# octavian-ganea/equidock_public

Measured on NVIDIA H100. Metric: protein_pairs_per_sec_iegmn_fwd_kabsch, higher is better.
Workload: dtype f32

## Files before the change

equidock_public_b200/csrc/attn_tc.cu:

```cuda
#include "tc_common.cuh"

namespace eqd {

#define AT_THREADS 256
#define AT_KEYS 64
#define AT_CHUNK_BYTES 8192
#define AT_A_SPLIT 16384
#define AT_LD 68

struct AtGroupSmem {
  unsigned char k[2][3][AT_CHUNK_BYTES];
  unsigned char v[2][3][AT_CHUNK_BYTES];
  float red[EQD_TM * 2];
  float x5c[2][AT_KEYS * 16];
  float red5[EQD_TM * 2 * 5];
};
struct AtSmem {
  unsigned char qa[3 * AT_A_SPLIT];
  unsigned char pa[3 * AT_A_SPLIT];
  AtGroupSmem grp;
  unsigned long long k_bar[2], v_bar[2];
};

__global__ void __launch_bounds__(AT_THREADS, 1)
attention0_tc_kernel(eqd_graph g, const float* __restrict__ proj, int pw, const unsigned char* __restrict__ kv,
                    long kv_split_stride, const float* __restrict__ x5, float* __restrict__ mu, int ldmu) {
  extern __shared__ __align__(128) unsigned char smem_raw[];
  AtSmem& S = *reinterpret_cast<AtSmem*>(smem_raw);
  const int tid = threadIdx.x, q = tid, half = q >> 7, r = q & 127, wgi = tid >> 7;
  AtGroupSmem& G = S.grp;
  if (tid == 0) {
    for (int b = 0; b < 2; ++b) {
      mbar_init(&S.k_bar[b], 1);
      mbar_init(&S.v_bar[b], 1);
    }
    asm volatile("fence.mbarrier_init.release.cluster;" ::: "memory");
  }
  __syncthreads();
  const unsigned k_saddr = smem_u32(G.k), v_saddr = smem_u32(G.v);
  const unsigned qa_saddr = smem_u32(S.qa), pa_saddr = smem_u32(S.pa);
  float* const dtile = reinterpret_cast<float*>(S.pa);
  unsigned kph[2] = {0, 0}, vph[2] = {0, 0};
  const int B = g.n_pairs;
  const unsigned char* k_g = kv;
  const unsigned char* v_g = kv + 3 * kv_split_stride;

  auto load_chunk = [&](const unsigned char* src, unsigned char (*dst)[AT_CHUNK_BYTES], unsigned long long* bar, int blk0,
                        int x5buf) {
    if (q == 0) {
      const bool with5 = x5buf >= 0;
      mbar_expect_tx(bar, 3 * AT_CHUNK_BYTES + (with5 ? AT_KEYS * 64 : 0));
#pragma unroll
      for (int s = 0; s < 3; ++s) bulk_g2s(dst[s], src + s * kv_split_stride + (long)blk0 * 1024, AT_CHUNK_BYTES, bar);
      if (with5) bulk_g2s(G.x5c[x5buf], x5 + (long)blk0 * 8 * 16, AT_KEYS * 64, bar);
    }
  };
  auto add_s5 = [&](float (&s)[32], const float* xc, const float (&q5)[5]) {
#pragma unroll
    for (int i = 0; i < 32; ++i) {
      const float* row = xc + (half * 32 + i) * 16;
      const float4 k4 = *reinterpret_cast<const float4*>(row);
      const float k8 = row[8];
      s[i] += q5[0] * k4.x + q5[1] * k4.y + q5[2] * k4.z + q5[3] * k4.w + q5[4] * k8;
    }
  };
  auto gemm_s = [&](int kb_, bool hi_only) {
    float d[32];
    wg_gemm6<64>(d, [&](int sp, int kb) { return a_desc_at<EQD_TM>(qa_saddr, AT_A_SPLIT, wgi, sp, kb); },
                 [&](int sp, int kk) { return b_desc_ex(k_saddr + (kb_ * 3 + sp) * AT_CHUNK_BYTES + kk * 256, 128, 1024); },
                 4, false, hi_only);
    wg_store_d<64>(dtile + wgi * 64 * AT_LD, AT_LD, d, tid & 127);
  };
  auto gemm_pv = [&](int vb_) {
    float d[32];
    wg_gemm6<64, 1>(d, [&](int sp, int kb) { return a_desc_at<EQD_TM>(pa_saddr, AT_A_SPLIT, wgi, sp, kb); },
                    [&](int sp, int kk) { return b_desc_ex(v_saddr + (vb_ * 3 + sp) * AT_CHUNK_BYTES + kk * 2048, 1024, 128); },
                    4, false);
    __syncthreads();
    wg_store_d<64>(dtile + wgi * 64 * AT_LD, AT_LD, d, tid & 127);
  };

  for (int tile = blockIdx.x; tile < g.n_node_tiles; tile += gridDim.x) {
    const int seg = g.node_tiles[2 * tile], node0 = g.node_tiles[2 * tile + 1];
    const int nvalid = min(EQD_TM, g.seg_ptr[seg + 1] - node0);
    const int pseg = seg < B ? seg + B : seg - B;
    const int j0 = g.seg_ptr[pseg], j1 = g.seg_ptr[pseg + 1];
    const int blk_lo = j0 >> 3, blk_hi = (j1 + 7) >> 3;
    const int nchunks = (blk_hi - blk_lo + 7) >> 3;
    const int node = node0 + r;
    const bool valid = r < nvalid;
    if (nchunks > 0) load_chunk(k_g, G.k[0], &S.k_bar[0], blk_lo, 0);
    float q5[5] = {0.f, 0.f, 0.f, 0.f, 0.f};
    if (valid) {
#pragma unroll
      for (int e = 0; e < 5; ++e) q5[e] = x5[(long)node * 16 + 10 + e];
    }
    {
      float v[32];
      const float4* sp = reinterpret_cast<const float4*>(proj + (long)node * pw + 128 + half * 32);
#pragma unroll
      for (int c4 = 0; c4 < 8; ++c4) {
        float4 t = valid ? sp[c4] : make_float4(0.f, 0.f, 0.f, 0.f);
        v[c4 * 4] = t.x; v[c4 * 4 + 1] = t.y; v[c4 * 4 + 2] = t.z; v[c4 * 4 + 3] = t.w;
      }
      store_half_split3<EQD_TM>(S.qa, AT_A_SPLIT, r, half * 32, v);
    }
    tc_fence_before();
    __syncthreads();
    float mx = -INFINITY;
    for (int c = 0; c < nchunks; ++c) {
      const int kb_ = c & 1;
      mbar_wait(&S.k_bar[kb_], kph[kb_]);
      kph[kb_] ^= 1;
      if (c + 1 < nchunks) load_chunk(k_g, G.k[kb_ ^ 1], &S.k_bar[kb_ ^ 1], blk_lo + 8 * (c + 1), kb_ ^ 1);
      else load_chunk(k_g, G.k[kb_ ^ 1], &S.k_bar[kb_ ^ 1], blk_lo, kb_ ^ 1);
      gemm_s(kb_, true);
      __syncthreads();
      float s[32];
      tile_ld32f(dtile, AT_LD, r, half * 32, s);
      add_s5(s, G.x5c[kb_], q5);
      const int key0 = (blk_lo + 8 * c) * 8 + half * 32;
#pragma unroll
      for (int i = 0; i < 32; ++i) {
        int kn = key0 + i;
        mx = fmaxf(mx, (kn >= j0 && kn < j1) ? s[i] : -INFINITY);
      }
      __syncthreads();
    }
    G.red[r * 2 + half] = mx;
    __syncthreads();
    mx = fmaxf(G.red[r * 2], G.red[r * 2 + 1]);
    float l = 0.f;
    float o_acc[32];
#pragma unroll
    for (int i = 0; i < 32; ++i) o_acc[i] = 0.f;
    if (nchunks > 0) load_chunk(v_g, G.v[0], &S.v_bar[0], blk_lo, -1);
    float o5[5] = {0.f, 0.f, 0.f, 0.f, 0.f};
    for (int c = 0; c < nchunks; ++c) {
      const int kb_ = (nchunks + c) & 1, vb_ = c & 1;
      mbar_wait(&S.k_bar[kb_], kph[kb_]);
      kph[kb_] ^= 1;
      if (c + 1 < nchunks) {
        load_chunk(k_g, G.k[kb_ ^ 1], &S.k_bar[kb_ ^ 1], blk_lo + 8 * (c + 1), kb_ ^ 1);
        load_chunk(v_g, G.v[vb_ ^ 1], &S.v_bar[vb_ ^ 1], blk_lo + 8 * (c + 1), -1);
      }
      gemm_s(kb_, false);
      __syncthreads();
      float s[32];
      tile_ld32f(dtile, AT_LD, r, half * 32, s);
      add_s5(s, G.x5c[kb_], q5);
      const int key0 = (blk_lo + 8 * c) * 8 + half * 32;
      float l4[4] = {0.f, 0.f, 0.f, 0.f};
#pragma unroll
      for (int i = 0; i < 32; ++i) {
        int kn = key0 + i;
        float pj = (kn >= j0 && kn < j1) ? expf(s[i] - mx) : 0.f;
        s[i] = pj;
        l4[i & 3] += pj;
        {
          const float* row = G.x5c[kb_] + (half * 32 + i) * 16;
          const float4 v4 = *reinterpret_cast<const float4*>(row + 4);
          o5[0] = fmaf(pj, v4.x, o5[0]);
          o5[1] = fmaf(pj, v4.y, o5[1]);
          o5[2] = fmaf(pj, v4.z, o5[2]);
          o5[3] = fmaf(pj, v4.w, o5[3]);
          o5[4] = fmaf(pj, row[9], o5[4]);
        }
      }
      l += (l4[0] + l4[1]) + (l4[2] + l4[3]);
      __syncthreads();
      store_half_split3<EQD_TM>(S.pa, AT_A_SPLIT, r, half * 32, s);
      tc_fence_before();
      __syncthreads();
      mbar_wait(&S.v_bar[vb_], vph[vb_]);
      vph[vb_] ^= 1;
      gemm_pv(vb_);
      __syncthreads();
      {
        float oc[32];
        tile_ld32f(dtile, AT_LD, r, half * 32, oc);
#pragma unroll
        for (int i = 0; i < 32; ++i) o_acc[i] += oc[i];
      }
      __syncthreads();
    }
    G.red[r * 2 + half] = l;
    {
#pragma unroll
      for (int e = 0; e < 5; ++e) G.red5[(r * 2 + half) * 5 + e] = o5[e];
    }
    __syncthreads();
    l = G.red[r * 2] + G.red[r * 2 + 1];
    {
      const float inv = l > 0.f ? 1.f / l : 0.f;
      if (valid && half == 0) {
        float e8[8];
#pragma unroll
        for (int e = 0; e < 5; ++e) e8[e] = (G.red5[r * 10 + e] + G.red5[r * 10 + 5 + e]) * inv;
        e8[5] = e8[6] = e8[7] = 0.f;
        float4* de = reinterpret_cast<float4*>(mu + (long)node * ldmu + 64);
        de[0] = make_float4(e8[0], e8[1], e8[2], e8[3]);
        de[1] = make_float4(e8[4], e8[5], e8[6], e8[7]);
      }
      if (valid) {
        float4* dst = reinterpret_cast<float4*>(mu + (long)node * ldmu + half * 32);
#pragma unroll
        for (int c4 = 0; c4 < 8; ++c4)
          dst[c4] = make_float4(o_acc[c4 * 4] * inv, o_acc[c4 * 4 + 1] * inv, o_acc[c4 * 4 + 2] * inv, o_acc[c4 * 4 + 3] * inv);
      }
    }
    __syncthreads();
  }
}

#define AT_CHAINS 2

struct __align__(128) AtChainSmem {
  unsigned char k[2][3][AT_CHUNK_BYTES];
  unsigned char v[2][3][AT_CHUNK_BYTES];
  float qs[64 * 64];
  unsigned long long k_bar[2], v_bar[2];
};

struct AtTile {
  int node0, nvalid;
  int j0, j1;
  int blk_lo, nchunks;
};

template <int P>
__global__ void __launch_bounds__(AT_CHAINS * 128, 1)
attention64_tc_kernel(eqd_graph g, const float* __restrict__ proj, const unsigned char* __restrict__ kv,
                      long kv_split_stride, float* __restrict__ mu) {
  extern __shared__ __align__(128) unsigned char smem_raw[];
  AtChainSmem& W = reinterpret_cast<AtChainSmem*>(smem_raw)[threadIdx.x >> 7];
  const int tid = threadIdx.x, wgi = tid >> 7, t = tid & 127, lane = t & 31;
  const int bar = 1 + wgi;
  if (t == 0) {
    for (int b = 0; b < 2; ++b) {
      mbar_init(&W.k_bar[b], 1);
      mbar_init(&W.v_bar[b], 1);
    }
    asm volatile("fence.mbarrier_init.release.cluster;" ::: "memory");
  }
  wg_barrier(bar);
  const unsigned k_saddr = smem_u32(W.k), v_saddr = smem_u32(W.v);
  const int B = g.n_pairs, nht = 2 * g.n_node_tiles, hstride = gridDim.x * AT_CHAINS;
  const unsigned char* k_g = kv;
  const unsigned char* v_g = kv + 3 * kv_split_stride;

  const int chain = blockIdx.x * AT_CHAINS + wgi;
  auto find_tile = [&](int k, AtTile& m) {
    for (; chain + k * hstride < nht; ++k) {
      const int ht = (chain + k * hstride) ^ (k & 1);
      const int seg = __ldg(g.node_tiles + 2 * (ht >> 1));
      m.node0 = __ldg(g.node_tiles + 2 * (ht >> 1) + 1) + 64 * (ht & 1);
      m.nvalid = min(64, __ldg(g.seg_ptr + seg + 1) - m.node0);
      if (m.nvalid <= 0) continue;
      const int pseg = seg < B ? seg + B : seg - B;
      m.j0 = __ldg(g.seg_ptr + pseg);
      m.j1 = __ldg(g.seg_ptr + pseg + 1);
      m.blk_lo = m.j0 >> 3;
      m.nchunks = (((m.j1 + 7) >> 3) - m.blk_lo + 7) >> 3;
      return k;
    }
    return -1;
  };
  unsigned kfill = 0, kcons = 0, vfill = 0, vcons = 0;
  auto fill = [&](unsigned char (*dst)[3][AT_CHUNK_BYTES], unsigned long long* bars, unsigned& n, const unsigned char* src,
                  int blk0) {
    if (t == 0) {
      unsigned long long* b = &bars[n & 1];
      mbar_expect_tx(b, 3 * AT_CHUNK_BYTES);
#pragma unroll
      for (int s = 0; s < 3; ++s) bulk_g2s(dst[n & 1][s], src + s * kv_split_stride + (long)blk0 * 1024, AT_CHUNK_BYTES, b);
    }
    ++n;
  };
  auto consume = [&](unsigned long long* bars, unsigned& n) {
    mbar_wait(&bars[n & 1], (n >> 1) & 1);
    return (int)((n++) & 1);
  };
  auto stage_q = [&](const AtTile& m) { stage_rows64(W.qs, proj, 320, 128, m.node0, m.nvalid, t); };

  const int fr0 = (t >> 5) * 16 + (lane >> 2), fc = 2 * (lane & 3);
  AtTile cur, nxt;
  int kt = find_tile(0, cur);
  bool k_ahead = false, v_ahead = false;
  if (kt >= 0) stage_q(cur);
  while (kt >= 0) {
    int ktn = -1;
    bool looked = false;
    auto look_ahead = [&]() {
      if (looked) return;
      looked = true;
      ktn = find_tile(kt + 1, nxt);
      if (ktn >= 0) stage_q(nxt);
    };
    if (cur.nchunks > 0 && !k_ahead) fill(W.k, W.k_bar, kfill, k_g, cur.blk_lo);
    cp_async_wait<0>();
    wg_barrier(bar);
    unsigned qf[3][4][4];
    staged_rows_to_a_split3<P>(W.qs, t, qf);
    wg_barrier(bar);
    auto k_desc = [&](int kb_) {
      return [&, kb_](int sp, int kk) { return b_desc_ex(k_saddr + (kb_ * 3 + sp) * AT_CHUNK_BYTES + kk * 256, 128, 1024); };
    };
    float mx[2] = {-INFINITY, -INFINITY};
    for (int c = 0; c < cur.nchunks; ++c) {
      const int kb_ = consume(W.k_bar, kcons);
      fill(W.k, W.k_bar, kfill, k_g, cur.blk_lo + (c + 1 < cur.nchunks ? 8 * (c + 1) : 0));
      float s[32];
      wg_gemm6_rs_issue<64, 4, 0, true>(s, qf, k_desc(kb_), false);
      look_ahead();
      wg_mma_wait(s);
      const int key0 = (cur.blk_lo + 8 * c) * 8 + fc;
#pragma unroll
      for (int j = 0; j < 8; ++j)
#pragma unroll
        for (int e = 0; e < 2; ++e) {
          const int kn = key0 + 8 * j + e;
          const bool ok = kn >= cur.j0 && kn < cur.j1;
#pragma unroll
          for (int h = 0; h < 2; ++h) mx[h] = fmaxf(mx[h], ok ? s[4 * j + 2 * h + e] : -INFINITY);
        }
      wg_barrier(bar);
    }
    look_ahead();
#pragma unroll
    for (int h = 0; h < 2; ++h) {
      mx[h] = fmaxf(mx[h], __shfl_xor_sync(0xffffffffu, mx[h], 1));
      mx[h] = fmaxf(mx[h], __shfl_xor_sync(0xffffffffu, mx[h], 2));
    }
    float lh[2][2] = {{0.f, 0.f}, {0.f, 0.f}};
    float o_acc[32];
#pragma unroll
    for (int i = 0; i < 32; ++i) o_acc[i] = 0.f;
    if (cur.nchunks > 0 && !v_ahead) fill(W.v, W.v_bar, vfill, v_g, cur.blk_lo);
    for (int c = 0; c < cur.nchunks; ++c) {
      const int kb_ = consume(W.k_bar, kcons);
      const bool last = c + 1 == cur.nchunks;
      if (!last) {
        fill(W.k, W.k_bar, kfill, k_g, cur.blk_lo + 8 * (c + 1));
        fill(W.v, W.v_bar, vfill, v_g, cur.blk_lo + 8 * (c + 1));
      } else if (ktn >= 0 && nxt.nchunks > 0) {
        fill(W.k, W.k_bar, kfill, k_g, nxt.blk_lo);
        fill(W.v, W.v_bar, vfill, v_g, nxt.blk_lo);
      }
      float s[32];
      wg_gemm6_rs_issue<64, 4, 0, false, P>(s, qf, k_desc(kb_), false);
      wg_mma_wait(s);
      const int key0 = (cur.blk_lo + 8 * c) * 8 + fc;
#pragma unroll
      for (int j = 0; j < 8; ++j)
#pragma unroll
        for (int e = 0; e < 2; ++e) {
          const int kn = key0 + 8 * j + e;
          const bool ok = kn >= cur.j0 && kn < cur.j1;
#pragma unroll
          for (int h = 0; h < 2; ++h) {
            float& x = s[4 * j + 2 * h + e];
            x = ok ? expf(x - mx[h]) : 0.f;
          }
        }
      {
        float ps[32];
#pragma unroll
        for (int i = 0; i < 32; ++i) ps[i] = __shfl_xor_sync(0xffffffffu, s[i], 2);
#pragma unroll
        for (int h = 0; h < 2; ++h)
#pragma unroll
          for (int ch = 0; ch < 2; ++ch) {
            float s0 = 0.f, s1 = 0.f;
#pragma unroll
            for (int c4 = 0; c4 < 8; ++c4) {
              s0 = __fadd_rn(s0, chain_val(s, ps, h, ch, c4, 0));
              s1 = __fadd_rn(s1, chain_val(s, ps, h, ch, c4, 1));
            }
            const float sp = __fadd_rn(s0, s1);
            lh[h][ch] = __fadd_rn(lh[h][ch], __fadd_rn(sp, __shfl_xor_sync(0xffffffffu, sp, 1)));
          }
      }
      unsigned pf[3][4][4];
      acc_to_a_split3<4, P>(s, pf);
      const int vb_ = consume(W.v_bar, vcons);
      float o[32];
      wg_gemm6_rs_issue<64, 4, 1, false, P>(o, pf, [&](int sp, int kk) {
        return b_desc_ex(v_saddr + (vb_ * 3 + sp) * AT_CHUNK_BYTES + kk * 2048, 1024, 128); }, false);
      wg_mma_wait(o);
#pragma unroll
      for (int i = 0; i < 32; ++i) o_acc[i] = __fadd_rn(o_acc[i], o[i]);
      wg_barrier(bar);
    }
    k_ahead = v_ahead = ktn >= 0 && nxt.nchunks > 0 && cur.nchunks > 0;
#pragma unroll
    for (int h = 0; h < 2; ++h) {
      const float l = __fadd_rn(lh[h][0], lh[h][1]);
      const float inv = l > 0.f ? 1.f / l : 0.f;
      const int row = fr0 + 8 * h;
      if (row < cur.nvalid) {
        float* dst = mu + (long)(cur.node0 + row) * EQD_HID + fc;
#pragma unroll
        for (int j = 0; j < 8; ++j)
          *reinterpret_cast<float2*>(dst + 8 * j) = make_float2(o_acc[4 * j + 2 * h] * inv, o_acc[4 * j + 2 * h + 1] * inv);
      }
    }
    kt = ktn;
    cur = nxt;
  }
  cp_async_wait<0>();
}

template <int P>
static int launch_attention64_tc(const eqd_graph* g, const float* proj, const void* kv, float* mu, void* stream) {
  const size_t smem = AT_CHAINS * sizeof(AtChainSmem);
  EQD_SET_SMEM(attention64_tc_kernel<P>, smem);
  const int nht = 2 * g->n_node_tiles;
  int grid = (nht + AT_CHAINS - 1) / AT_CHAINS;
  if (grid > EQD_SMS) grid = EQD_SMS;
  const long split_stride = (long)((g->n_nodes + 7) / 8 + 8) * 1024;
  attention64_tc_kernel<P><<<grid, AT_CHAINS * 128, smem, (cudaStream_t)stream>>>(
      *g, proj, reinterpret_cast<const unsigned char*>(kv), split_stride, mu);
  EQD_CUDA_LAUNCH_CHECK();
  return EQD_OK;
}

}

int eqd_attention_tc_products(const eqd_graph* g, const float* proj, const void* kv, float* mu, int products, void* stream) {
  if (!g || !proj || !kv || !mu) return EQD_ERR_BAD_ARG;
  if (reinterpret_cast<uintptr_t>(kv) & 15) return EQD_ERR_BAD_ARG;
  if (products != 6 && products != 3) return EQD_ERR_UNSUPPORTED;
  if (g->n_node_tiles <= 0) return EQD_OK;
  return products == 3 ? eqd::launch_attention64_tc<3>(g, proj, kv, mu, stream)
                       : eqd::launch_attention64_tc<6>(g, proj, kv, mu, stream);
}

extern "C" int eqd_attention_tc(const eqd_graph* g, const float* proj, const void* kv, float* mu, void* stream) {
  return eqd_attention_tc_products(g, proj, kv, mu, 6, stream);
}

extern "C" int eqd_attention_tc0(const eqd_graph* g, const float* proj, const void* kv, const float* x5, float* mu,
                                 void* stream) {
  if (!g || !proj || !kv || !x5 || !mu) return EQD_ERR_BAD_ARG;
  if ((reinterpret_cast<uintptr_t>(kv) | reinterpret_cast<uintptr_t>(x5)) & 15) return EQD_ERR_BAD_ARG;
  if (g->n_node_tiles <= 0) return EQD_OK;
  const size_t smem = sizeof(eqd::AtSmem) + 128;
  EQD_SET_SMEM(eqd::attention0_tc_kernel, smem);
  const int grid = g->n_node_tiles < EQD_SMS ? g->n_node_tiles : EQD_SMS;
  const long split_stride = (long)((g->n_nodes + 7) / 8 + 8) * 1024;
  eqd::attention0_tc_kernel<<<grid, AT_THREADS, smem, (cudaStream_t)stream>>>(
      *g, proj, 128 + 3 * 72, reinterpret_cast<const unsigned char*>(kv), split_stride, x5, mu, EQD_H0_PAD);
  EQD_CUDA_LAUNCH_CHECK();
  return EQD_OK;
}
```

equidock_public_b200/csrc/tc_common.cuh:

```cuda
#pragma once
#include "common.cuh"

namespace eqd {

__device__ __forceinline__ unsigned smem_u32(const void* p) { return (unsigned)__cvta_generic_to_shared(p); }

__device__ __forceinline__ void mbar_init(unsigned long long* bar, int count) {
  asm volatile("mbarrier.init.shared::cta.b64 [%0], %1;" ::"r"(smem_u32(bar)), "r"(count));
}
__device__ __forceinline__ void mbar_wait(unsigned long long* bar, unsigned parity) {
  unsigned addr = smem_u32(bar);
  unsigned done = 0;
  while (!done) {
    asm volatile(
        "{\n\t.reg .pred p;\n\t"
        "mbarrier.try_wait.parity.shared::cta.b64 p, [%1], %2;\n\t"
        "selp.u32 %0, 1, 0, p;\n\t}"
        : "=r"(done) : "r"(addr), "r"(parity) : "memory");
  }
}
__device__ __forceinline__ void mbar_expect_tx(unsigned long long* bar, unsigned bytes) {
  asm volatile("mbarrier.arrive.expect_tx.shared::cta.b64 _, [%0], %1;" ::"r"(smem_u32(bar)), "r"(bytes) : "memory");
}
__device__ __forceinline__ void bulk_g2s(void* dst, const void* src, unsigned bytes, unsigned long long* bar) {
  asm volatile("cp.async.bulk.shared::cluster.global.mbarrier::complete_tx::bytes [%0], [%1], %2, [%3];" ::"r"(smem_u32(dst)),
               "l"(src), "r"(bytes), "r"(smem_u32(bar)) : "memory");
}
__device__ __forceinline__ void cp_async8(void* dst, const void* src) {
  asm volatile("cp.async.ca.shared.global [%0], [%1], 8;" ::"r"(smem_u32(dst)), "l"(src));
}
__device__ __forceinline__ void cp_async4(void* dst, const void* src) {
  asm volatile("cp.async.ca.shared.global [%0], [%1], 4;" ::"r"(smem_u32(dst)), "l"(src));
}
__device__ __forceinline__ void tc_fence_before() { asm volatile("fence.proxy.async.shared::cta;" ::: "memory"); }

__device__ __forceinline__ unsigned long long b_desc_ex(unsigned saddr, unsigned lbo, unsigned sbo) {
  return (unsigned long long)((saddr >> 4) & 0x3FFF) | ((unsigned long long)((lbo >> 4) & 0x3FFF) << 16) |
         ((unsigned long long)((sbo >> 4) & 0x3FFF) << 32);
}

template <int N, int TB>
struct Wgmma;
template <int TB>
struct Wgmma<16, TB> {
  static __device__ __forceinline__ void mma(float (&d)[8], unsigned long long a, unsigned long long b, int scale_d) {
    asm volatile(
        "{\n\t.reg .pred p;\n\tsetp.ne.b32 p, %10, 0;\n\t"
        "wgmma.mma_async.sync.aligned.m64n16k16.f32.bf16.bf16 {%0, %1, %2, %3, %4, %5, %6, %7}, %8, %9, p, 1, 1, 0, %11;\n\t}"
        : "+f"(d[0]), "+f"(d[1]), "+f"(d[2]), "+f"(d[3]), "+f"(d[4]), "+f"(d[5]), "+f"(d[6]), "+f"(d[7])
        : "l"(a), "l"(b), "r"(scale_d), "n"(TB));
  }
};
template <int TB>
struct Wgmma<64, TB> {
  static __device__ __forceinline__ void mma(float (&d)[32], unsigned long long a, unsigned long long b, int scale_d) {
    asm volatile(
        "{\n\t.reg .pred p;\n\tsetp.ne.b32 p, %34, 0;\n\t"
        "wgmma.mma_async.sync.aligned.m64n64k16.f32.bf16.bf16 {%0, %1, %2, %3, %4, %5, %6, %7, %8, %9, %10, %11, %12, %13, %14, %15, %16, %17, %18, %19, %20, %21, %22, %23, %24, %25, %26, %27, %28, %29, %30, %31}, %32, %33, p, 1, 1, 0, %35;\n\t}"
        : "+f"(d[0]), "+f"(d[1]), "+f"(d[2]), "+f"(d[3]), "+f"(d[4]), "+f"(d[5]), "+f"(d[6]), "+f"(d[7]), "+f"(d[8]), "+f"(d[9]), "+f"(d[10]), "+f"(d[11]), "+f"(d[12]), "+f"(d[13]), "+f"(d[14]), "+f"(d[15]), "+f"(d[16]), "+f"(d[17]), "+f"(d[18]), "+f"(d[19]), "+f"(d[20]), "+f"(d[21]), "+f"(d[22]), "+f"(d[23]), "+f"(d[24]), "+f"(d[25]), "+f"(d[26]), "+f"(d[27]), "+f"(d[28]), "+f"(d[29]), "+f"(d[30]), "+f"(d[31])
        : "l"(a), "l"(b), "r"(scale_d), "n"(TB));
  }
};
template <int TB>
struct Wgmma<80, TB> {
  static __device__ __forceinline__ void mma(float (&d)[40], unsigned long long a, unsigned long long b, int scale_d) {
    asm volatile(
        "{\n\t.reg .pred p;\n\tsetp.ne.b32 p, %42, 0;\n\t"
        "wgmma.mma_async.sync.aligned.m64n80k16.f32.bf16.bf16 {%0, %1, %2, %3, %4, %5, %6, %7, %8, %9, %10, %11, %12, %13, %14, %15, %16, %17, %18, %19, %20, %21, %22, %23, %24, %25, %26, %27, %28, %29, %30, %31, %32, %33, %34, %35, %36, %37, %38, %39}, %40, %41, p, 1, 1, 0, %43;\n\t}"
        : "+f"(d[0]), "+f"(d[1]), "+f"(d[2]), "+f"(d[3]), "+f"(d[4]), "+f"(d[5]), "+f"(d[6]), "+f"(d[7]), "+f"(d[8]), "+f"(d[9]), "+f"(d[10]), "+f"(d[11]), "+f"(d[12]), "+f"(d[13]), "+f"(d[14]), "+f"(d[15]), "+f"(d[16]), "+f"(d[17]), "+f"(d[18]), "+f"(d[19]), "+f"(d[20]), "+f"(d[21]), "+f"(d[22]), "+f"(d[23]), "+f"(d[24]), "+f"(d[25]), "+f"(d[26]), "+f"(d[27]), "+f"(d[28]), "+f"(d[29]), "+f"(d[30]), "+f"(d[31]), "+f"(d[32]), "+f"(d[33]), "+f"(d[34]), "+f"(d[35]), "+f"(d[36]), "+f"(d[37]), "+f"(d[38]), "+f"(d[39])
        : "l"(a), "l"(b), "r"(scale_d), "n"(TB));
  }
};

template <int N, int TB>
struct WgmmaRS;
template <int TB>
struct WgmmaRS<64, TB> {
  static __device__ __forceinline__ void mma(float (&d)[32], const unsigned (&a)[4], unsigned long long b, int scale_d) {
    asm volatile(
        "{\n\t.reg .pred p;\n\tsetp.ne.b32 p, %37, 0;\n\t"
        "wgmma.mma_async.sync.aligned.m64n64k16.f32.bf16.bf16 {%0, %1, %2, %3, %4, %5, %6, %7, %8, %9, %10, %11, %12, %13, %14, %15, %16, %17, %18, %19, %20, %21, %22, %23, %24, %25, %26, %27, %28, %29, %30, %31}, {%32, %33, %34, %35}, %36, p, 1, 1, %38;\n\t}"
        : "+f"(d[0]), "+f"(d[1]), "+f"(d[2]), "+f"(d[3]), "+f"(d[4]), "+f"(d[5]), "+f"(d[6]), "+f"(d[7]), "+f"(d[8]), "+f"(d[9]), "+f"(d[10]), "+f"(d[11]), "+f"(d[12]), "+f"(d[13]), "+f"(d[14]), "+f"(d[15]), "+f"(d[16]), "+f"(d[17]), "+f"(d[18]), "+f"(d[19]), "+f"(d[20]), "+f"(d[21]), "+f"(d[22]), "+f"(d[23]), "+f"(d[24]), "+f"(d[25]), "+f"(d[26]), "+f"(d[27]), "+f"(d[28]), "+f"(d[29]), "+f"(d[30]), "+f"(d[31])
        : "r"(a[0]), "r"(a[1]), "r"(a[2]), "r"(a[3]), "l"(b), "r"(scale_d), "n"(TB));
  }
};

template <int N, int TB = 0, int P = 6, class AD, class BD>
__device__ __forceinline__ void wg_gemm6_issue(float (&d)[N / 2], AD a_desc, BD b_desc, int kblocks, bool accumulate,
                                               bool hi_only = false) {
  static_assert(P == 6 || P == 3, "bf16x6 or bf16x3");
  const int pa[6] = {2, 0, 1, 1, 0, 0}, pb[6] = {0, 2, 1, 0, 1, 0};
  asm volatile("wgmma.fence.sync.aligned;" ::: "memory");
  int scale_d = accumulate ? 1 : 0;
#pragma unroll
  for (int pr = hi_only ? 5 : 6 - P; pr < 6; ++pr)
    for (int kb = 0; kb < kblocks; ++kb) {
      Wgmma<N, TB>::mma(d, a_desc(pa[pr], kb), b_desc(pb[pr], kb), scale_d);
      scale_d = 1;
    }
  asm volatile("wgmma.commit_group.sync.aligned;" ::: "memory");
}
template <int PENDING = 0, int M>
__device__ __forceinline__ void wg_mma_wait(float (&d)[M]) {
  asm volatile("wgmma.wait_group.sync.aligned %0;" ::"n"(PENDING) : "memory");
#pragma unroll
  for (int i = 0; i < M; ++i) asm volatile("" : "+f"(d[i])::"memory");
}
template <int N, int TB = 0, int P = 6, class AD, class BD>
__device__ __forceinline__ void wg_gemm6(float (&d)[N / 2], AD a_desc, BD b_desc, int kblocks, bool accumulate,
                                         bool hi_only = false) {
  wg_gemm6_issue<N, TB, P>(d, a_desc, b_desc, kblocks, accumulate, hi_only);
  asm volatile("wgmma.wait_group.sync.aligned 0;" ::: "memory");
}
template <int N, int KB, int TB = 0, bool HI_ONLY = false, int P = 6, class BD>
__device__ __forceinline__ void wg_gemm6_rs_issue(float (&d)[N / 2], const unsigned (&a)[3][KB][4], BD b_desc, bool accumulate) {
  static_assert(P == 6 || P == 3, "bf16x6 or bf16x3");
  constexpr int pa[6] = {2, 0, 1, 1, 0, 0}, pb[6] = {0, 2, 1, 0, 1, 0};
  asm volatile("wgmma.fence.sync.aligned;" ::: "memory");
  int scale_d = accumulate ? 1 : 0;
#pragma unroll
  for (int pr = HI_ONLY ? 5 : 6 - P; pr < 6; ++pr)
#pragma unroll
    for (int kb = 0; kb < KB; ++kb) {
      WgmmaRS<N, TB>::mma(d, a[pa[pr]][kb], b_desc(pb[pr], kb), scale_d);
      scale_d = 1;
    }
  asm volatile("wgmma.commit_group.sync.aligned;" ::: "memory");
}

template <int R>
__device__ __forceinline__ unsigned long long a_desc_at(unsigned a_saddr, unsigned split_bytes, int wgi, int s, int kb) {
  return b_desc_ex(a_saddr + s * split_bytes + kb * (32 * R) + wgi * 1024, 16 * R, 128);
}
template <int R, int P = 6>
__device__ __forceinline__ void a_store8(unsigned char* a, unsigned split_bytes, int row, int c, const unsigned* p0,
                                         const unsigned* p1, const unsigned* p2) {
  unsigned char* base = a + (c >> 4) * (32 * R) + ((c >> 3) & 1) * (16 * R) + (row >> 3) * 128 + (row & 7) * 16;
  *reinterpret_cast<uint4*>(base) = make_uint4(p0[0], p0[1], p0[2], p0[3]);
  *reinterpret_cast<uint4*>(base + split_bytes) = make_uint4(p1[0], p1[1], p1[2], p1[3]);
  if constexpr (P == 6) *reinterpret_cast<uint4*>(base + 2 * split_bytes) = make_uint4(p2[0], p2[1], p2[2], p2[3]);
}

template <int N>
__device__ __forceinline__ void wg_store_d(float* tile, int ld, const float (&d)[N / 2], int t) {
  const int row = (t >> 5) * 16 + ((t & 31) >> 2), col = 2 * (t & 3);
#pragma unroll
  for (int j = 0; j < N / 8; ++j) {
    *reinterpret_cast<float2*>(tile + row * ld + 8 * j + col) = make_float2(d[4 * j], d[4 * j + 1]);
    *reinterpret_cast<float2*>(tile + (row + 8) * ld + 8 * j + col) = make_float2(d[4 * j + 2], d[4 * j + 3]);
  }
}

__device__ __forceinline__ unsigned cvt_bf16x2(float hi, float lo) {
  unsigned d;
  asm("cvt.rn.bf16x2.f32 %0, %1, %2;" : "=r"(d) : "f"(hi), "f"(lo));
  return d;
}
template <int P = 6>
__device__ __forceinline__ void split3_pair(float v0, float v1, unsigned& p0, unsigned& p1, unsigned& p2) {
  p0 = cvt_bf16x2(v1, v0);
  const float r0 = v0 - __uint_as_float(p0 << 16), r1 = v1 - __uint_as_float(p0 & 0xFFFF0000u);
  p1 = cvt_bf16x2(r1, r0);
  if constexpr (P == 6) p2 = cvt_bf16x2(r1 - __uint_as_float(p1 & 0xFFFF0000u), r0 - __uint_as_float(p1 << 16));
}
template <int R>
__device__ __forceinline__ void store_half_split3(unsigned char* a, unsigned split_bytes, int row, int c0, const float (&v)[32]) {
  unsigned p0[16], p1[16], p2[16];
#pragma unroll
  for (int c = 0; c < 16; ++c) split3_pair(v[2 * c], v[2 * c + 1], p0[c], p1[c], p2[c]);
#pragma unroll
  for (int j = 0; j < 4; ++j) a_store8<R>(a, split_bytes, row, c0 + 8 * j, p0 + 4 * j, p1 + 4 * j, p2 + 4 * j);
}
template <int R>
__device__ __forceinline__ void store_extra8_split3(unsigned char* a, unsigned split_bytes, int row, int c0, const float (&t)[8]) {
  unsigned p0[8], p1[8], p2[8];
#pragma unroll
  for (int c = 0; c < 4; ++c) split3_pair(t[2 * c], t[2 * c + 1], p0[c], p1[c], p2[c]);
#pragma unroll
  for (int c = 4; c < 8; ++c) p0[c] = p1[c] = p2[c] = 0u;
  a_store8<R>(a, split_bytes, row, c0, p0, p1, p2);
  a_store8<R>(a, split_bytes, row, c0 + 8, p0 + 4, p1 + 4, p2 + 4);
}
template <int KB, int P = 6>
__device__ __forceinline__ void acc_to_a_split3(const float (&v)[8 * KB], unsigned (&a)[3][KB][4]) {
#pragma unroll
  for (int kb = 0; kb < KB; ++kb)
#pragma unroll
    for (int i = 0; i < 4; ++i) split3_pair<P>(v[8 * kb + 2 * i], v[8 * kb + 2 * i + 1], a[0][kb][i], a[1][kb][i], a[2][kb][i]);
}
__device__ __forceinline__ int stage_swz(int row) { return (row & 3) << 1; }
__device__ __forceinline__ void stage_rows64(float* rows, const float* src, int ld, int col0, long row0, int nvalid, int t) {
#pragma unroll
  for (int i = 0; i < 8; ++i) {
    const int idx = i * 128 + t, row = idx >> 4, k4 = idx & 15;
    const bool ok = row < nvalid;
    cp_async16(rows + row * 64 + ((k4 ^ stage_swz(row)) << 2), src + (row0 + (ok ? row : 0)) * ld + col0 + 4 * k4, ok);
  }
  cp_async_commit();
}
template <int P = 6>
__device__ __forceinline__ void staged_rows_to_a_split3(const float* rows, int t, unsigned (&a)[3][4][4]) {
  const int g = (t >> 5) * 16 + ((t & 31) >> 2), c = t & 3;
#pragma unroll
  for (int kb = 0; kb < 4; ++kb)
#pragma unroll
    for (int i = 0; i < 4; ++i) {
      const int row = g + 8 * (i & 1), k4 = 4 * kb + 2 * (i >> 1) + (c >> 1);
      const float2 v = *reinterpret_cast<const float2*>(rows + row * 64 + ((k4 ^ stage_swz(row)) << 2) + 2 * (c & 1));
      split3_pair<P>(v.x, v.y, a[0][kb][i], a[1][kb][i], a[2][kb][i]);
    }
}
__device__ __forceinline__ void staged_rows_to_frag(const float* rows, int t, float (&v)[32]) {
  const int g = (t >> 5) * 16 + ((t & 31) >> 2), c = t & 3;
#pragma unroll
  for (int kb = 0; kb < 4; ++kb)
#pragma unroll
    for (int i = 0; i < 4; ++i) {
      const int row = g + 8 * (i & 1), k4 = 4 * kb + 2 * (i >> 1) + (c >> 1);
      const float2 x = *reinterpret_cast<const float2*>(rows + row * 64 + ((k4 ^ stage_swz(row)) << 2) + 2 * (c & 1));
      v[8 * kb + 2 * i] = x.x;
      v[8 * kb + 2 * i + 1] = x.y;
    }
}
__device__ __forceinline__ float chain_val(const float (&v)[32], const float (&pv)[32], int h, int ch, int c4, int e) {
  const int i = 4 * (4 * ch + (c4 >> 1)) + 2 * h + e;
  const bool own = ((c4 & 1) == 0) == ((threadIdx.x & 2) == 0);
  return own ? v[i] : pv[i];
}
__device__ __forceinline__ void wg_barrier(int id) { asm volatile("bar.sync %0, 128;" ::"r"(id) : "memory"); }
__device__ __forceinline__ bool wg_barrier_and(int id, bool pred) {
  unsigned all;
  asm volatile(
      "{\n\t.reg .pred p, q;\n\tsetp.ne.u32 p, %1, 0;\n\t"
      "bar.red.and.pred q, %2, 128, p;\n\tselp.u32 %0, 1, 0, q;\n\t}"
      : "=r"(all) : "r"((unsigned)pred), "r"(id) : "memory");
  return all != 0;
}
__device__ __forceinline__ void tile_ld32f(const float* tile, int ld, int row, int c0, float (&v)[32]) {
  const float4* s = reinterpret_cast<const float4*>(tile + row * ld + c0);
#pragma unroll
  for (int c4 = 0; c4 < 8; ++c4) {
    float4 t = s[c4];
    v[c4 * 4] = t.x; v[c4 * 4 + 1] = t.y; v[c4 * 4 + 2] = t.z; v[c4 * 4 + 3] = t.w;
  }
}

__device__ __forceinline__ void quad_ln_stats(const float (&v)[32], float (&mean)[2], float (&rstd)[2]) {
  float pv[32];
#pragma unroll
  for (int i = 0; i < 32; ++i) pv[i] = __shfl_xor_sync(0xffffffffu, v[i], 2);
#pragma unroll
  for (int h = 0; h < 2; ++h) {
    float mh[2], qh[2];
#pragma unroll
    for (int ch = 0; ch < 2; ++ch) {
      float s0 = 0.f, s1 = 0.f;
#pragma unroll
      for (int c4 = 0; c4 < 8; ++c4) {
        s0 = __fadd_rn(s0, chain_val(v, pv, h, ch, c4, 0));
        s1 = __fadd_rn(s1, chain_val(v, pv, h, ch, c4, 1));
      }
      const float sp = s0 + s1;
      mh[ch] = (sp + __shfl_xor_sync(0xffffffffu, sp, 1)) * (1.f / 32.f);
      float q0 = 0.f, q1 = 0.f;
#pragma unroll
      for (int c4 = 0; c4 < 8; ++c4) {
        const float d0 = __fadd_rn(chain_val(v, pv, h, ch, c4, 0), -mh[ch]);
        const float d1 = __fadd_rn(chain_val(v, pv, h, ch, c4, 1), -mh[ch]);
        q0 = fmaf(d0, d0, q0);
        q1 = fmaf(d1, d1, q1);
      }
      const float qp = q0 + q1;
      qh[ch] = qp + __shfl_xor_sync(0xffffffffu, qp, 1);
    }
    const float m0 = mh[0], m1 = mh[1];
    mean[h] = 0.5f * (m0 + m1);
    const float dm = m0 - m1;
    const float var = (qh[0] + qh[1] + dm * dm * 16.f) * (1.f / 64.f);
    rstd[h] = 1.f / sqrtf(var + 1e-5f);
  }
}

__device__ __forceinline__ void quad_ln_apply(float (&v)[32], const float (&mean)[2], const float (&rstd)[2],
                                              const float* ln_g, const float* ln_b, int fc) {
#pragma unroll
  for (int j = 0; j < 8; ++j) {
    const float2 gj = *reinterpret_cast<const float2*>(&ln_g[8 * j + fc]);
    const float2 bj = *reinterpret_cast<const float2*>(&ln_b[8 * j + fc]);
#pragma unroll
    for (int h = 0; h < 2; ++h) {
      float& x0 = v[4 * j + 2 * h];
      float& x1 = v[4 * j + 2 * h + 1];
      x0 = fmaf(__fmul_rn(__fadd_rn(x0, -mean[h]), rstd[h]), gj.x, bj.x);
      x1 = fmaf(__fmul_rn(__fadd_rn(x1, -mean[h]), rstd[h]), gj.y, bj.y);
    }
  }
}

}
```

Baseline: 43080.

## Share K/V ring across chains with 3-stage full/empty mbarriers and variable-width chunks

Both warpgroups in a block now work on the two halves of the same node tile. They share one 3-stage K/V shared-memory ring guarded by full/empty mbarriers, so each chunk of keys and values is loaded once per block instead of once per chain. Partial tail chunks use narrower wgmma shapes (n8/n16/n32) and copy fewer bytes. Fewer splits are fetched where the precision mode allows it. This cuts duplicate bulk copies and wasted MMA work on small proteins, at the cost of coupling the two chains through shared barriers and adding more template instantiations.

```diff
diff --git a/equidock_public_b200/csrc/attn_tc.cu b/equidock_public_b200/csrc/attn_tc.cu
--- a/equidock_public_b200/csrc/attn_tc.cu
+++ b/equidock_public_b200/csrc/attn_tc.cu
@@ -214,79 +214,115 @@
 }
 
 #define AT_CHAINS 2
-
-struct __align__(128) AtChainSmem {
-  unsigned char k[2][3][AT_CHUNK_BYTES];
-  unsigned char v[2][3][AT_CHUNK_BYTES];
-  float qs[64 * 64];
-  unsigned long long k_bar[2], v_bar[2];
+#define AT_STAGES 3
+
+struct __align__(128) At64Smem {
+  unsigned char k[AT_STAGES][3][AT_CHUNK_BYTES];
+  unsigned char v[AT_STAGES][3][AT_CHUNK_BYTES];
+  float qs[AT_CHAINS][64 * 64];
+  unsigned long long k_full[AT_STAGES], k_empty[AT_STAGES], v_full[AT_STAGES], v_empty[AT_STAGES];
 };
 
 struct AtTile {
   int node0, nvalid;
   int j0, j1;
-  int blk_lo, nchunks;
+  int blk_lo, nblk;
+  int nchunks;
 };
+
+__device__ __forceinline__ int at_chunk_blocks(int nblk, int c) {
+  const int left = nblk - 8 * c;
+  return left >= 5 ? 8 : left >= 3 ? 4 : left;
+}
+template <int NB>
+struct AtNb {
+  static constexpr int value = NB;
+};
+template <class F>
+__device__ __forceinline__ void at_with_blocks(int nb, F&& f) {
+  if (nb == 8) f(AtNb<8>());
+  else if (nb == 4) f(AtNb<4>());
+  else if (nb == 2) f(AtNb<2>());
+  else f(AtNb<1>());
+}
 
 template <int P>
 __global__ void __launch_bounds__(AT_CHAINS * 128, 1)
 attention64_tc_kernel(eqd_graph g, const float* __restrict__ proj, const unsigned char* __restrict__ kv,
                       long kv_split_stride, float* __restrict__ mu) {
+  constexpr int SPLITS2 = P == 3 ? 2 : 3;
   extern __shared__ __align__(128) unsigned char smem_raw[];
-  AtChainSmem& W = reinterpret_cast<AtChainSmem*>(smem_raw)[threadIdx.x >> 7];
+  At64Smem& W = *reinterpret_cast<At64Smem*>(smem_raw);
   const int tid = threadIdx.x, wgi = tid >> 7, t = tid & 127, lane = t & 31;
   const int bar = 1 + wgi;
-  if (t == 0) {
-    for (int b = 0; b < 2; ++b) {
-      mbar_init(&W.k_bar[b], 1);
-      mbar_init(&W.v_bar[b], 1);
+  if (tid == 0) {
+    for (int b = 0; b < AT_STAGES; ++b) {
+      mbar_init(&W.k_full[b], 1);
+      mbar_init(&W.v_full[b], 1);
+      mbar_init(&W.k_empty[b], AT_CHAINS);
+      mbar_init(&W.v_empty[b], AT_CHAINS);
     }
     asm volatile("fence.mbarrier_init.release.cluster;" ::: "memory");
   }
-  wg_barrier(bar);
+  __syncthreads();
   const unsigned k_saddr = smem_u32(W.k), v_saddr = smem_u32(W.v);
-  const int B = g.n_pairs, nht = 2 * g.n_node_tiles, hstride = gridDim.x * AT_CHAINS;
+  float* const qs = W.qs[wgi];
+  const int B = g.n_pairs;
   const unsigned char* k_g = kv;
   const unsigned char* v_g = kv + 3 * kv_split_stride;
 
-  const int chain = blockIdx.x * AT_CHAINS + wgi;
   auto find_tile = [&](int k, AtTile& m) {
-    for (; chain + k * hstride < nht; ++k) {
-      const int ht = (chain + k * hstride) ^ (k & 1);
-      const int seg = __ldg(g.node_tiles + 2 * (ht >> 1));
-      m.node0 = __ldg(g.node_tiles + 2 * (ht >> 1) + 1) + 64 * (ht & 1);
-      m.nvalid = min(64, __ldg(g.seg_ptr + seg + 1) - m.node0);
-      if (m.nvalid <= 0) continue;
-      const int pseg = seg < B ? seg + B : seg - B;
-      m.j0 = __ldg(g.seg_ptr + pseg);
-      m.j1 = __ldg(g.seg_ptr + pseg + 1);
-      m.blk_lo = m.j0 >> 3;
-      m.nchunks = (((m.j1 + 7) >> 3) - m.blk_lo + 7) >> 3;
-      return k;
-    }
-    return -1;
+    const int nt = blockIdx.x + k * gridDim.x;
+    if (nt >= g.n_node_tiles) return -1;
+    const int seg = __ldg(g.node_tiles + 2 * nt);
+    m.node0 = __ldg(g.node_tiles + 2 * nt + 1) + 64 * wgi;
+    m.nvalid = min(64, __ldg(g.seg_ptr + seg + 1) - m.node0);
+    const int pseg = seg < B ? seg + B : seg - B;
+    m.j0 = __ldg(g.seg_ptr + pseg);
+    m.j1 = __ldg(g.seg_ptr + pseg + 1);
+    m.blk_lo = m.j0 >> 3;
+    m.nblk = ((m.j1 + 7) >> 3) - m.blk_lo;
+    m.nchunks = (m.nblk + 7) >> 3;
+    return k;
   };
   unsigned kfill = 0, kcons = 0, vfill = 0, vcons = 0;
-  auto fill = [&](unsigned char (*dst)[3][AT_CHUNK_BYTES], unsigned long long* bars, unsigned& n, const unsigned char* src,
-                  int blk0) {
-    if (t == 0) {
-      unsigned long long* b = &bars[n & 1];
-      mbar_expect_tx(b, 3 * AT_CHUNK_BYTES);
-#pragma unroll
-      for (int s = 0; s < 3; ++s) bulk_g2s(dst[n & 1][s], src + s * kv_split_stride + (long)blk0 * 1024, AT_CHUNK_BYTES, b);
+  auto fill = [&](unsigned char (*ring)[3][AT_CHUNK_BYTES], unsigned long long* full, unsigned long long* empty,
+                  unsigned& n, const unsigned char* src, int blk0, int nblocks, int nsplits) {
+    if (tid == 0) {
+      const unsigned st = n % AT_STAGES;
+      if (n >= AT_STAGES) mbar_wait(&empty[st], (n / AT_STAGES + 1) & 1);
+      mbar_expect_tx(&full[st], nsplits * nblocks * 1024);
+      for (int s = 0; s < nsplits; ++s)
+        bulk_g2s(ring[st][s], src + s * kv_split_stride + (long)blk0 * 1024, nblocks * 1024, &full[st]);
     }
     ++n;
   };
-  auto consume = [&](unsigned long long* bars, unsigned& n) {
-    mbar_wait(&bars[n & 1], (n >> 1) & 1);
-    return (int)((n++) & 1);
-  };
-  auto stage_q = [&](const AtTile& m) { stage_rows64(W.qs, proj, 320, 128, m.node0, m.nvalid, t); };
+  auto fill_k = [&](const AtTile& m, int c, int nsplits) {
+    fill(W.k, W.k_full, W.k_empty, kfill, k_g, m.blk_lo + 8 * c, at_chunk_blocks(m.nblk, c), nsplits);
+  };
+  auto fill_v = [&](const AtTile& m, int c) {
+    fill(W.v, W.v_full, W.v_empty, vfill, v_g, m.blk_lo + 8 * c, max(2, at_chunk_blocks(m.nblk, c)), SPLITS2);
+  };
+  auto consume = [&](unsigned long long* full, unsigned& n) {
+    const unsigned st = n % AT_STAGES;
+    mbar_wait(&full[st], (n / AT_STAGES) & 1);
+    ++n;
+    return (int)st;
+  };
+  auto release = [&](unsigned long long* empty, int st) {
+    if (t == 0) mbar_arrive(&empty[st]);
+  };
+  auto stage_q = [&](const AtTile& m) {
+    if (m.nvalid > 0) stage_rows64(qs, proj, 320, 128, m.node0, m.nvalid, t);
+  };
+  auto k_desc = [&](int st) {
+    return [&, st](int sp, int kk) { return b_desc_ex(k_saddr + (st * 3 + sp) * AT_CHUNK_BYTES + kk * 256, 128, 1024); };
+  };
 
   const int fr0 = (t >> 5) * 16 + (lane >> 2), fc = 2 * (lane & 3);
   AtTile cur, nxt;
   int kt = find_tile(0, cur);
-  bool k_ahead = false, v_ahead = false;
+  bool ahead = false;
   if (kt >= 0) stage_q(cur);
   while (kt >= 0) {
     int ktn = -1;
@@ -297,34 +333,37 @@
       ktn = find_tile(kt + 1, nxt);
       if (ktn >= 0) stage_q(nxt);
     };
-    if (cur.nchunks > 0 && !k_ahead) fill(W.k, W.k_bar, kfill, k_g, cur.blk_lo);
+    const bool live = cur.nvalid > 0;
+    if (cur.nchunks > 0 && !ahead) fill_k(cur, 0, 1);
     cp_async_wait<0>();
     wg_barrier(bar);
     unsigned qf[3][4][4];
-    staged_rows_to_a_split3<P>(W.qs, t, qf);
+    if (live) staged_rows_to_a_split3<P>(qs, t, qf);
     wg_barrier(bar);
-    auto k_desc = [&](int kb_) {
-      return [&, kb_](int sp, int kk) { return b_desc_ex(k_saddr + (kb_ * 3 + sp) * AT_CHUNK_BYTES + kk * 256, 128, 1024); };
-    };
     float mx[2] = {-INFINITY, -INFINITY};
     for (int c = 0; c < cur.nchunks; ++c) {
-      const int kb_ = consume(W.k_bar, kcons);
-      fill(W.k, W.k_bar, kfill, k_g, cur.blk_lo + (c + 1 < cur.nchunks ? 8 * (c + 1) : 0));
-      float s[32];
-      wg_gemm6_rs_issue<64, 4, 0, true>(s, qf, k_desc(kb_), false);
-      look_ahead();
-      wg_mma_wait(s);
-      const int key0 = (cur.blk_lo + 8 * c) * 8 + fc;
-#pragma unroll
-      for (int j = 0; j < 8; ++j)
-#pragma unroll
-        for (int e = 0; e < 2; ++e) {
-          const int kn = key0 + 8 * j + e;
-          const bool ok = kn >= cur.j0 && kn < cur.j1;
-#pragma unroll
-          for (int h = 0; h < 2; ++h) mx[h] = fmaxf(mx[h], ok ? s[4 * j + 2 * h + e] : -INFINITY);
-        }
+      const int st = consume(W.k_full, kcons);
+      if (c + 1 < cur.nchunks) fill_k(cur, c + 1, 1);
+      else fill_k(cur, 0, SPLITS2);
+      if (live) at_with_blocks(at_chunk_blocks(cur.nblk, c), [&](auto nbc) {
+        constexpr int NB = decltype(nbc)::value;
+        float s[4 * NB];
+        wg_gemm6_rs_issue<8 * NB, 4, 0, true>(s, qf, k_desc(st), false);
+        look_ahead();
+        wg_mma_wait(s);
+        const int key0 = (cur.blk_lo + 8 * c) * 8 + fc;
+#pragma unroll
+        for (int j = 0; j < NB; ++j)
+#pragma unroll
+          for (int e = 0; e < 2; ++e) {
+            const int kn = key0 + 8 * j + e;
+            const bool ok = kn >= cur.j0 && kn < cur.j1;
+#pragma unroll
+            for (int h = 0; h < 2; ++h) mx[h] = fmaxf(mx[h], ok ? s[4 * j + 2 * h + e] : -INFINITY);
+          }
+      });
       wg_barrier(bar);
+      release(W.k_empty, st);
     }
     look_ahead();
 #pragma unroll
@@ -336,63 +375,74 @@
     float o_acc[32];
 #pragma unroll
     for (int i = 0; i < 32; ++i) o_acc[i] = 0.f;
-    if (cur.nchunks > 0 && !v_ahead) fill(W.v, W.v_bar, vfill, v_g, cur.blk_lo);
+    if (cur.nchunks > 0 && !ahead) fill_v(cur, 0);
     for (int c = 0; c < cur.nchunks; ++c) {
-      const int kb_ = consume(W.k_bar, kcons);
-      const bool last = c + 1 == cur.nchunks;
-      if (!last) {
-        fill(W.k, W.k_bar, kfill, k_g, cur.blk_lo + 8 * (c + 1));
-        fill(W.v, W.v_bar, vfill, v_g, cur.blk_lo + 8 * (c + 1));
+      const int kst = consume(W.k_full, kcons);
+      if (c + 1 < cur.nchunks) {
+        fill_k(cur, c + 1, SPLITS2);
+        fill_v(cur, c + 1);
       } else if (ktn >= 0 && nxt.nchunks > 0) {
-        fill(W.k, W.k_bar, kfill, k_g, nxt.blk_lo);
-        fill(W.v, W.v_bar, vfill, v_g, nxt.blk_lo);
-      }
-      float s[32];
-      wg_gemm6_rs_issue<64, 4, 0, false, P>(s, qf, k_desc(kb_), false);
-      wg_mma_wait(s);
-      const int key0 = (cur.blk_lo + 8 * c) * 8 + fc;
-#pragma unroll
-      for (int j = 0; j < 8; ++j)
-#pragma unroll
-        for (int e = 0; e < 2; ++e) {
-          const int kn = key0 + 8 * j + e;
-          const bool ok = kn >= cur.j0 && kn < cur.j1;
-#pragma unroll
-          for (int h = 0; h < 2; ++h) {
-            float& x = s[4 * j + 2 * h + e];
-            x = ok ? expf(x - mx[h]) : 0.f;
+        fill_k(nxt, 0, 1);
+        fill_v(nxt, 0);
+      }
+      int vst;
+      if (live) at_with_blocks(at_chunk_blocks(cur.nblk, c), [&](auto nbc) {
+        constexpr int NB = decltype(nbc)::value, KBV = (NB + 1) / 2;
+        float s[4 * NB];
+        wg_gemm6_rs_issue<8 * NB, 4, 0, false, P>(s, qf, k_desc(kst), false);
+        wg_mma_wait(s);
+        const int key0 = (cur.blk_lo + 8 * c) * 8 + fc;
+#pragma unroll
+        for (int j = 0; j < NB; ++j)
+#pragma unroll
+          for (int e = 0; e < 2; ++e) {
+            const int kn = key0 + 8 * j + e;
+            const bool ok = kn >= cur.j0 && kn < cur.j1;
+#pragma unroll
+            for (int h = 0; h < 2; ++h) {
+              float& x = s[4 * j + 2 * h + e];
+              x = ok ? expf(x - mx[h]) : 0.f;
+            }
           }
+        {
+          float ps[4 * NB];
+#pragma unroll
+          for (int i = 0; i < 4 * NB; ++i) ps[i] = __shfl_xor_sync(0xffffffffu, s[i], 2);
+#pragma unroll
+          for (int h = 0; h < 2; ++h)
+#pragma unroll
+            for (int ch = 0; ch < 2; ++ch) {
+              if (4 * ch >= NB) continue;
+              float s0 = 0.f, s1 = 0.f;
+#pragma unroll
+              for (int c4 = 0; c4 < 8; ++c4) {
+                if (4 * ch + (c4 >> 1) >= NB) continue;
+                s0 = __fadd_rn(s0, chain_val(s, ps, h, ch, c4, 0));
+                s1 = __fadd_rn(s1, chain_val(s, ps, h, ch, c4, 1));
+              }
+              const float sp = __fadd_rn(s0, s1);
+              lh[h][ch] = __fadd_rn(lh[h][ch], __fadd_rn(sp, __shfl_xor_sync(0xffffffffu, sp, 1)));
+            }
         }
-      {
-        float ps[32];
-#pragma unroll
-        for (int i = 0; i < 32; ++i) ps[i] = __shfl_xor_sync(0xffffffffu, s[i], 2);
-#pragma unroll
-        for (int h = 0; h < 2; ++h)
-#pragma unroll
-          for (int ch = 0; ch < 2; ++ch) {
-            float s0 = 0.f, s1 = 0.f;
-#pragma unroll
-            for (int c4 = 0; c4 < 8; ++c4) {
-              s0 = __fadd_rn(s0, chain_val(s, ps, h, ch, c4, 0));
-              s1 = __fadd_rn(s1, chain_val(s, ps, h, ch, c4, 1));
-            }
-            const float sp = __fadd_rn(s0, s1);
-            lh[h][ch] = __fadd_rn(lh[h][ch], __fadd_rn(sp, __shfl_xor_sync(0xffffffffu, sp, 1)));
-          }
-      }
-      unsigned pf[3][4][4];
-      acc_to_a_split3<4, P>(s, pf);
-      const int vb_ = consume(W.v_bar, vcons);
-      float o[32];
-      wg_gemm6_rs_issue<64, 4, 1, false, P>(o, pf, [&](int sp, int kk) {
-        return b_desc_ex(v_saddr + (vb_ * 3 + sp) * AT_CHUNK_BYTES + kk * 2048, 1024, 128); }, false);
-      wg_mma_wait(o);
-#pragma unroll
-      for (int i = 0; i < 32; ++i) o_acc[i] = __fadd_rn(o_acc[i], o[i]);
+        float p[8 * KBV];
+#pragma unroll
+        for (int i = 0; i < 8 * KBV; ++i) p[i] = i < 4 * NB ? s[i] : 0.f;
+        unsigned pf[3][KBV][4];
+        acc_to_a_split3<KBV, P>(p, pf);
+        vst = consume(W.v_full, vcons);
+        float o[32];
+        wg_gemm6_rs_issue<64, KBV, 1, false, P>(o, pf, [&](int sp, int kk) {
+          return b_desc_ex(v_saddr + (vst * 3 + sp) * AT_CHUNK_BYTES + kk * 2048, 1024, 128); }, false);
+        wg_mma_wait(o);
+#pragma unroll
+        for (int i = 0; i < 32; ++i) o_acc[i] = __fadd_rn(o_acc[i], o[i]);
+      });
+      else vst = consume(W.v_full, vcons);
       wg_barrier(bar);
-    }
-    k_ahead = v_ahead = ktn >= 0 && nxt.nchunks > 0 && cur.nchunks > 0;
+      release(W.k_empty, kst);
+      release(W.v_empty, vst);
+    }
+    ahead = ktn >= 0 && nxt.nchunks > 0 && cur.nchunks > 0;
 #pragma unroll
     for (int h = 0; h < 2; ++h) {
       const float l = __fadd_rn(lh[h][0], lh[h][1]);
@@ -413,11 +463,9 @@
 
 template <int P>
 static int launch_attention64_tc(const eqd_graph* g, const float* proj, const void* kv, float* mu, void* stream) {
-  const size_t smem = AT_CHAINS * sizeof(AtChainSmem);
+  const size_t smem = sizeof(At64Smem);
   EQD_SET_SMEM(attention64_tc_kernel<P>, smem);
-  const int nht = 2 * g->n_node_tiles;
-  int grid = (nht + AT_CHAINS - 1) / AT_CHAINS;
-  if (grid > EQD_SMS) grid = EQD_SMS;
+  const int grid = g->n_node_tiles < EQD_SMS ? g->n_node_tiles : EQD_SMS;
   const long split_stride = (long)((g->n_nodes + 7) / 8 + 8) * 1024;
   attention64_tc_kernel<P><<<grid, AT_CHAINS * 128, smem, (cudaStream_t)stream>>>(
       *g, proj, reinterpret_cast<const unsigned char*>(kv), split_stride, mu);
diff --git a/equidock_public_b200/csrc/tc_common.cuh b/equidock_public_b200/csrc/tc_common.cuh
--- a/equidock_public_b200/csrc/tc_common.cuh
+++ b/equidock_public_b200/csrc/tc_common.cuh
@@ -19,6 +19,9 @@
         : "=r"(done) : "r"(addr), "r"(parity) : "memory");
   }
 }
+__device__ __forceinline__ void mbar_arrive(unsigned long long* bar) {
+  asm volatile("mbarrier.arrive.shared::cta.b64 _, [%0];" ::"r"(smem_u32(bar)) : "memory");
+}
 __device__ __forceinline__ void mbar_expect_tx(unsigned long long* bar, unsigned bytes) {
   asm volatile("mbarrier.arrive.expect_tx.shared::cta.b64 _, [%0], %1;" ::"r"(smem_u32(bar)), "r"(bytes) : "memory");
 }
@@ -74,6 +77,36 @@
 
 template <int N, int TB>
 struct WgmmaRS;
+template <int TB>
+struct WgmmaRS<8, TB> {
+  static __device__ __forceinline__ void mma(float (&d)[4], const unsigned (&a)[4], unsigned long long b, int scale_d) {
+    asm volatile(
+        "{\n\t.reg .pred p;\n\tsetp.ne.b32 p, %9, 0;\n\t"
+        "wgmma.mma_async.sync.aligned.m64n8k16.f32.bf16.bf16 {%0, %1, %2, %3}, {%4, %5, %6, %7}, %8, p, 1, 1, %10;\n\t}"
+        : "+f"(d[0]), "+f"(d[1]), "+f"(d[2]), "+f"(d[3])
+        : "r"(a[0]), "r"(a[1]), "r"(a[2]), "r"(a[3]), "l"(b), "r"(scale_d), "n"(TB));
+  }
+};
+template <int TB>
+struct WgmmaRS<16, TB> {
+  static __device__ __forceinline__ void mma(float (&d)[8], const unsigned (&a)[4], unsigned long long b, int scale_d) {
+    asm volatile(
+        "{\n\t.reg .pred p;\n\tsetp.ne.b32 p, %13, 0;\n\t"
+        "wgmma.mma_async.sync.aligned.m64n16k16.f32.bf16.bf16 {%0, %1, %2, %3, %4, %5, %6, %7}, {%8, %9, %10, %11}, %12, p, 1, 1, %14;\n\t}"
+        : "+f"(d[0]), "+f"(d[1]), "+f"(d[2]), "+f"(d[3]), "+f"(d[4]), "+f"(d[5]), "+f"(d[6]), "+f"(d[7])
+        : "r"(a[0]), "r"(a[1]), "r"(a[2]), "r"(a[3]), "l"(b), "r"(scale_d), "n"(TB));
+  }
+};
+template <int TB>
+struct WgmmaRS<32, TB> {
+  static __device__ __forceinline__ void mma(float (&d)[16], const unsigned (&a)[4], unsigned long long b, int scale_d) {
+    asm volatile(
+        "{\n\t.reg .pred p;\n\tsetp.ne.b32 p, %21, 0;\n\t"
+        "wgmma.mma_async.sync.aligned.m64n32k16.f32.bf16.bf16 {%0, %1, %2, %3, %4, %5, %6, %7, %8, %9, %10, %11, %12, %13, %14, %15}, {%16, %17, %18, %19}, %20, p, 1, 1, %22;\n\t}"
+        : "+f"(d[0]), "+f"(d[1]), "+f"(d[2]), "+f"(d[3]), "+f"(d[4]), "+f"(d[5]), "+f"(d[6]), "+f"(d[7]), "+f"(d[8]), "+f"(d[9]), "+f"(d[10]), "+f"(d[11]), "+f"(d[12]), "+f"(d[13]), "+f"(d[14]), "+f"(d[15])
+        : "r"(a[0]), "r"(a[1]), "r"(a[2]), "r"(a[3]), "l"(b), "r"(scale_d), "n"(TB));
+  }
+};
 template <int TB>
 struct WgmmaRS<64, TB> {
   static __device__ __forceinline__ void mma(float (&d)[32], const unsigned (&a)[4], unsigned long long b, int scale_d) {
@@ -222,7 +255,8 @@
       v[8 * kb + 2 * i + 1] = x.y;
     }
 }
-__device__ __forceinline__ float chain_val(const float (&v)[32], const float (&pv)[32], int h, int ch, int c4, int e) {
+template <int M>
+__device__ __forceinline__ float chain_val(const float (&v)[M], const float (&pv)[M], int h, int ch, int c4, int e) {
   const int i = 4 * (4 * ch + (c4 >> 1)) + 2 * h + e;
   const bool own = ((c4 & 1) == 0) == ((threadIdx.x & 2) == 0);
   return own ? v[i] : pv[i];
```

New measurement: 44340, median of 6. 1.03x the previous value.
